# abdur75648/AI-Camera

Hardware: AMD Instinct MI355X
Metric: end-to-end frames/sec @1280x720, 30 persons/frame (higher is better)
Workload: dtype f16

## Files before the change

### ai-camera_amd/_lib.py

```python
from __future__ import annotations

import ctypes as C
import os

import numpy as np

HERE = os.path.dirname(os.path.abspath(__file__))
LIB_PATH = os.path.join(HERE, "libaicam.so")

OK, ERR_INVALID, ERR_NOT_FOUND, ERR_RUNTIME, ERR_NO_DEVICE, ERR_CAPACITY, ERR_FORMAT = 0, -1, -2, -3, -4, -5, -6
HOST, DEVICE = 0, 1
F32, F16 = 0, 1
MODEL_YOLO, MODEL_REID = 1, 2
PIX_BGR24, PIX_NV12, PIX_I420 = 0, 1, 2
YUV_BT601, YUV_BT709 = 0, 1
YUV_LIMITED, YUV_FULL = 0, 1
PROF_CLASSES = ("conv_igemm", "conv_direct", "misc", "letterbox", "crop_resize", "decode_nms", "tracker")


class AicError(RuntimeError):
    def __init__(self, code, msg):
        super().__init__(f"libaicam error {code}: {msg}")
        self.code = code

# ... 71 lines not shown
                ("max_persons", C.c_int32), ("conf_thresh", C.c_float), ("iou_thresh", C.c_float),
                ("max_det", C.c_int32), ("min_confidence", C.c_float), ("inject", C.c_int32),
                ("track_class_mask", C.c_uint64 * 2), ("tracker", TrackerParams)]


_P = C.c_void_p
_I = C.c_int
_F = C.c_float
_D = C.c_double
_SIGS = {
    "aic_last_error": (C.c_char_p, []),
    "aic_abi_version": (_I, []),
    "aic_device_count": (_I, [_P]),
    "aic_device_sync": (_I, [_I]),
    "aic_model_load": (_I, [C.c_char_p, _I, _I, _I, _P]),
    "aic_model_load_mem": (_I, [_P, C.c_size_t, _I, _I, _I, _P]),
    "aic_model_read_buffer": (_I, [_P, _I, _P, C.c_size_t]),
    "aic_model_conv_plan": (_I, [_P, _I, _I, _P]),
    "aic_model_conv_plan_live": (_I, [_P, _I, _I, _P]),
    "aic_model_row_band": (_I, [_P, _I, _I, _I, _P]),
    "aic_model_sparse_box": (_I, [_P, _I, _P]),
    "aic_debug_alloc_probe": (_I, [_I, _P, _P, _P, _P]),
    "aic_model_read_det": (_I, [_P, _I, _P, _P, _P]),
    "aic_detect_decode": (_I, [_P, _I, _I, _I, _F, _F, _I, _P, _P, _P, _P]),
    "aic_detect_live": (_I, [_P, _P, _I, _I, _I, _I, _I, _F, _F, _I, _P, _P, _P, _P]),
    "aic_model_destroy": (_I, [_P]),
    "aic_model_info": (_I, [_P, _P, _P, _P, _P, _P, _P, _P]),
    "aic_yolo_infer": (_I, [_P, _P, _I, _I, _F, _F, _I, _P, _P, _P, _P]),
    "aic_yolo_head": (_I, [_P, _P, _I, _I, _P, _P]),
    "aic_yolo_decode": (_I, [_P, _P, _I, _I, _P, _P, _P]),
    "aic_yolo_postprocess": (_I, [_P, _P, _P, _I, _F, _F, _I, _I, _F, _F, _F, _I, _I] + [_P] * 9),
    "aic_det_filter": (_I, [_I, _P, _P, _P, _P, _I, _I, _F, _P, _I] + [_P] * 9),
    "aic_reid_infer": (_I, [_P, _P, _I, _I, _P, _I]),
    "aic_reid_infer_live": (_I, [_P, _P, _I, _I, _I, _P, _I]),
    "aic_letterbox": (_I, [_I, _P, _I, _I, _I, _I, _P, _P, _P, _P]),
    "aic_letterbox_image": (_I, [_I, _P, _I, _I, _I, _I, _I, _I, _I, _I, _I, _I, _I, _P]),
    "aic_crop_resize": (_I, [_I, _P, _I, _I, _P, _I, _I, _I, _P, _P]),
    "aic_detect": (_I, [_P, _P, _I, _I, _I, _I, _F, _F, _I, _P, _P, _P, _P]),
    "aic_reid_embed": (_I, [_P, _P, _I, _I, _I, _P, _I, _P, _P]),
    "aic_crop_resize_ex": (_I, [_I, _P, _I, _I, _I, _I, _P, _P, _I, _I, _I, _I, _I, _I, _I, _P, _P]),
    "aic_reid_embed_bank": (_I, [_P, _P, _I, _I, _I, _I, _P, _P, _I, _I, _P, _P]),
    "aic_kf_initiate": (_I, [_I, _P, _I, _P, _P]),
    "aic_kf_predict": (_I, [_I, _P, _P, _I]),
    "aic_kf_predict_dt": (_I, [_I, _P, _P, _I, _F]),
    "aic_kf_project": (_I, [_I, _P, _P, _I, _P, _P]),
    "aic_kf_update": (_I, [_I, _P, _P, _P, _I]),
    "aic_kf_gating": (_I, [_I, _P, _P, _I, _P, _I, _I, _I, _P]),
    "aic_iou_cost": (_I, [_I, _P, _I, _P, _I, _P]),
    "aic_appearance_cost": (_I, [_I, _P, _P, _I, _I, _I, _P, _P, _I, _P]),
    "aic_lsap": (_I, [_P, _I, _I, _P, _P]),
    "aic_min_cost_matching": (_I, [_P, _I, _I, _D, _P, _P, _P]),
    "aic_match_cascade": (_I, [_P, _P, _P, _I, _I, _P, _P, _D, _D, _I, _P, _P, _P, _P, _P, _P, _P]),
    "aic_match_cascade_device": (_I, [_I, _P, _P, _P, _I, _I, _P, _P, _D, _D, _I, _I, _P, _P]),
    "aic_tracker_option": (_I, [_P, C.c_char_p, _I]),
    "aic_tracker_create": (_I, [_I, _P, _P]),
    "aic_tracker_destroy": (_I, [_P]),
    "aic_tracker_predict": (_I, [_P]),
    "aic_tracker_update": (_I, [_P, _P, _P, _P, _P, _I, _P, _I, _I]),
    "aic_tracker_update_batch": (_I, [_P, _I, _P, _P, _P, _P, _P, _I, _P, _I, _I, _P, _P, _P, _P, _P, _P]),
    "aic_tracker_import_state": (_I, [_P, _I, _P, _P, _P, _P, _P, _P, _P, _P, _P, _P, _P, _I, _I]),
    "aic_tracker_next_track_id": (_I, [_P, _P]),
    "aic_tracker_assoc_counters": (_I, [_P, _P, _P]),
    "aic_tracker_outputs": (_I, [_P, _P, _P, _I, _P]),
    "aic_tracker_num_tracks": (_I, [_P, _P]),
    "aic_tracker_export": (_I, [_P, _I, _P, _P, _P, _P, _P, _P, _P, _P, _P, _P]),
    "aic_tracker_export_gallery": (_I, [_P, _I, _P, _I]),
    "aic_tracker_last_matches": (_I, [_P, _P, _P, _I, _P]),
    "aic_tracker_last_costs": (_I, [_P, _P, _P, _P, _I, _P, _P]),
    "aic_pipeline_create": (_I, [_P, _P, _P, _P]),
    "aic_pipeline_destroy": (_I, [_P]),
    "aic_pipeline_upload": (_I, [_P, _I, _P, _I]),
    "aic_pipeline_inject": (_I, [_P, _I, _I, _P, _P, _P, _P]),
    "aic_pipeline_run": (_I, [_P, _I, _I, _P, _P, _P, _P, _P, _P, _P]),
    "aic_pipeline_run_passes": (_I, [_P, _I, _I, _I, _P, _P, _P, _P]),
    "aic_pipeline_run_from_host": (_I, [_P, _P, _I, _I, _P, _P, _P, _P]),
    "aic_pipeline_run_from_host_passes": (_I, [_P, _P, _I, _I, _I, _P, _P, _P, _P]),
    "aic_pipeline_group_times": (_I, [_P, _P, _P, _P, _I, _P]),
    "aic_pipeline_exchange_enable": (_I, [_P, _P, _P, _I, _I]),
    "aic_pipeline_exchange_stream": (_I, [_P, _P]),
    "aic_pipeline_exchange_wait": (_I, [_P, C.c_int64, _I, _P, _P]),
    "aic_pipeline_exchange_done": (_I, [_P, C.c_int64]),
    "aic_gallery_annotate": (_I, [_I, _P, _P, _I, _I, _I, _I, _D, _P, _P, _P, _P]),
    "aic_gid_create": (_I, [_I, _P]),
    "aic_gid_destroy": (_I, [_P]),
    "aic_gid_update": (_I, [_P, _I, _I, _P, _P, _P, _D, _P]),
    "aic_gid_lookup": (_I, [_P, _I, _I, _P]),
    "aic_gid_size": (_I, [_P, _P, _P, _P]),
    "aic_host_register": (_I, [_P, C.c_size_t]),
    "aic_host_unregister": (_I, [_P]),
    "aic_pipeline_tracker": (_I, [_P, _P]),
    "aic_pipeline_stats": (_I, [_P, _P, _P, _P, _P, _I]),
    "aic_pipeline_last_embeddings": (_I, [_P, _P, _I, _P, _P]),
    "aic_pipeline_option": (_I, [_P, C.c_char_p, _I]),
    "aic_pipeline_counters": (_I, [_P, _P, _P]),
    "aic_pipeline_assoc_frames": (_I, [_P, _P, _P]),
    "aic_pipeline_filter_counters": (_I, [_P, _P, _P, _P]),
    "aic_pipeline_lane_groups": (_I, [_P, _P]),
    "aic_pipeline_group_embeddings": (_I, [_P, _P, _I, _P, _I, _P, _P, _P]),
    "aic_overlay": (_I, [_I, _P, _I, _I, _I, _P, _I, _P, _I]),
    "aic_prof_enable": (_I, [_I, _I]),
    "aic_prof_reset": (_I, [_I]),
    "aic_prof_read": (_I, [_I, _I, _P, _P, _P, _P]),
    "aic_prof_read_union": (_I, [_I, _I, _P]),
    "aic_bytetrack_create": (_I, [_I, _P, _P]),
    "aic_bytetrack_destroy": (_I, [_P]),
    "aic_bytetrack_option": (_I, [_P, C.c_char_p, _I]),
# ... 239 lines not shown
```

### ai-camera_amd/csrc/kernels_trk_dev.hip

```cpp
#include "kernels.hpp"
#include "trk_dev.hpp"
#include "trk_math.hpp"
#include "trk_wave.hpp"

#include <algorithm>
#include <cstdio>
#include <cstdlib>

namespace aic {

namespace {

constexpr float kInfty = 1e5f;
constexpr float kChi2_4 = (float)9.487729036781154;
constexpr float kBig = 3.0e38f;

}

constexpr int SMG = 7;

__global__ __launch_bounds__(256) void trk_epoch_prep_kernel(const DevTrkHdr* __restrict__ hdr, const DevTrack* __restrict__ trk,
                                                             const float* __restrict__ gal_n, int gmax, int dim,
                                                             const float* __restrict__ featn, int dn, int dn_pad, int k,
                                                             float* __restrict__ sm, float* __restrict__ gram, int f0, EpochBankArgs bk) {
// ... 70 lines not shown
                        floatx4 a[4];
#pragma unroll
                        for (int u = 0; u < 4; ++u) a[u] = *reinterpret_cast<const floatx4*>(grow[g] + k0 + 16 * u + 4 * q);
#pragma unroll
                        for (int u = 0; u < 4; ++u)
#pragma unroll
                            for (int e = 0; e < 4; ++e) {
                                acc[g][0] = __builtin_amdgcn_mfma_f32_16x16x4f32(a[u][e], b0[u][e], acc[g][0], 0, 0, 0);
                                acc[g][1] = __builtin_amdgcn_mfma_f32_16x16x4f32(a[u][e], b1[u][e], acc[g][1], 0, 0, 0);
                            }
                    }
                }
            }
            for (; k0 < dim; k0 += 16) {
                const int kk = k0 + 4 * q;
                floatx4 b0 = {0.f, 0.f, 0.f, 0.f}, b1 = b0;
#pragma unroll
                for (int e = 0; e < 4; ++e)
                    if (kk + e < dim) { b0[e] = pa[kk + e]; b1[e] = pb[kk + e]; }
#pragma unroll
                for (int g = 0; g < SMG; ++g) {
                    if (g < ng) {
                        floatx4 a = {0.f, 0.f, 0.f, 0.f};
#pragma unroll
                        for (int e = 0; e < 4; ++e)
                            if (kk + e < dim) a[e] = grow[g][kk + e];
#pragma unroll
                        for (int e = 0; e < 4; ++e) {
                            acc[g][0] = __builtin_amdgcn_mfma_f32_16x16x4f32(a[e], b0[e], acc[g][0], 0, 0, 0);
                            acc[g][1] = __builtin_amdgcn_mfma_f32_16x16x4f32(a[e], b1[e], acc[g][1], 0, 0, 0);
                        }
                    }
                }
            }
#pragma unroll
            for (int g = SMG - 1; g >= 0; --g) {
                if (g < ng) {
#pragma unroll
                    for (int e = 0; e < 4; ++e) {
                        tile[4 * q + e][r] = cos_dist(acc[g][0][e]);
                        tile[4 * q + e][16 + r] = cos_dist(acc[g][1][e]);
                    }
                    wave_lds_sync();
                    if (lane < 32) {
                        for (int jj = 15; jj >= 0; --jj) {
                            const int row = 16 * (gb + g) + jj;
                            if (row < glen0) {
                                R = fminf(R, tile[jj][lane]);
                                if (row <= k) smt[(size_t)row * dn_pad + lane] = R;
                            }
                        }
                    }
                    wave_lds_sync();
                }
            }
        }
    }
}

namespace {

struct Lds {
    int *id, *state, *hits, *age, *tsu, *cls, *slot, *glen, *ghead, *sm, *napp, *glen0;
    float* conf;
    unsigned short* newrow;
    int ks;
    int *mdet;
    int *feas;
    float* tbox;
    int* free_slots;
    float *tlwh, *xyah, *dconf;
    int *dcls, *dhas, *mtrk, *und, *cols;
    int* rows;
    double *u, *v, *dist;
    int *pred, *rowof, *colof, *todo, *pos, *asg;
    int* wcnt;
    float* kf;
    float* arena;
    int arena_floats;
};

constexpr int KF_SLOTS = 96;

__device__ __forceinline__ Lds lds_carve(char* base, int cap, int nmax, int total_bytes, int ks = TRK_KMAX) {
    Lds L;
    char* p = base;
    auto take = [&](size_t bytes) { char* q = p; p += (bytes + 15) & ~(size_t)15; return q; };
    const size_t tc = (size_t)cap, mx = (size_t)max(cap, nmax);
    L.u = (double*)take(8 * mx); L.v = (double*)take(8 * mx); L.dist = (double*)take(8 * mx);
    int** ti[] = {&L.id, &L.state, &L.hits, &L.age, &L.tsu, &L.cls, &L.slot, &L.glen, &L.ghead, &L.sm, &L.napp, &L.glen0, &L.mdet, &L.rows, &L.feas};
    for (auto a : ti) *a = (int*)take(4 * tc);
    int** li[] = {&L.pred, &L.rowof, &L.colof, &L.todo, &L.pos, &L.asg};
    for (auto a : li) *a = (int*)take(4 * mx);
    L.conf = (float*)take(4 * tc);
    L.tbox = (float*)take(16 * tc);
    L.ks = ks;
    L.newrow = (unsigned short*)take(2 * tc * (size_t)ks);
    L.free_slots = (int*)take(4 * tc);
    L.kf = (float*)take(4 * 72 * (size_t)KF_SLOTS);
    L.tlwh = (float*)take(16 * (size_t)nmax); L.xyah = (float*)take(16 * (size_t)nmax); L.dconf = (float*)take(4 * (size_t)nmax);
    int** di[] = {&L.dcls, &L.dhas, &L.mtrk, &L.und, &L.cols};
    for (auto a : di) *a = (int*)take(4 * (size_t)nmax);
    L.wcnt = (int*)take(4 * (NW + 8));
    L.arena = (float*)p;
    L.arena_floats = (int)((total_bytes - (p - base)) / 4);
    return L;
// ... 858 lines not shown
    unsigned long long best = ~0ull;
    for (int j = tid; j < n; j += 256) {
        if (j / t_max == ri) continue;
        const float* gj = g + (size_t)j * w;
        if (!(gj[0] > 0.5f)) continue;
        float dot = 0.f;
        int k = 0;
        for (; k + 2 <= dim; k += 2) {
            const float2 b = *reinterpret_cast<const float2*>(gj + 2 + k);
            dot = dot + s_e[k] * b.x;
            dot = dot + s_e[k + 1] * b.y;
        }
        for (; k < dim; ++k) dot = dot + s_e[k] * gj[2 + k];
        const float d = cos_dist(dot);
        const unsigned long long key = ((unsigned long long)__float_as_uint(d) << 32) | (unsigned)j;
        best = key < best ? key : best;
    }
#pragma unroll
    for (int o = 32; o > 0; o >>= 1) {
        const unsigned long long other = __shfl_xor(best, o);
        best = other < best ? other : best;
    }
    if (lane == 0) s_best[wv] = best;
    __syncthreads();
    if (tid == 0) {
        unsigned long long b = s_best[0];
        for (int q = 1; q < 4; ++q) b = s_best[q] < b ? s_best[q] : b;
        near_row[i] = b == ~0ull ? -1 : (int)(unsigned)b;
        near_dist[i] = b == ~0ull ? kInfty : __uint_as_float((unsigned)(b >> 32));
    }
}

void launch_gallery_nearest(const float* gathered, int world, int t_max, int dim, int* ids, int* near_row, float* near_dist, hipStream_t s) {
    if (world * t_max <= 0) return;
    hipLaunchKernelGGL(gallery_nearest_kernel, dim3(world * t_max), dim3(256), (size_t)dim * 4, s, gathered, world, t_max, dim, ids, near_row, near_dist);
    KCHECK();
}

void launch_gallery_shard(const DevTrkHdr* hdr, const DevTrack* trk, const float* gal_n, int gmax, int dim, float* out, int t_max, hipStream_t s) {
    hipLaunchKernelGGL(gallery_shard_kernel, dim3(1), dim3(TRK_DEV_TMAX), 0, s, hdr, trk, gal_n, gmax, dim, out, t_max);
    KCHECK();
}

__global__ __launch_bounds__(256) void gallery_commit_kernel(const int* __restrict__ appends, const float* __restrict__ feat, const float* __restrict__ feat_n,
                                                             int d_begin, int dim, int gmax, float* __restrict__ gal_raw, float* __restrict__ gal_n,
                                                             size_t gal_stride) {
    appends += (size_t)blockIdx.y * TRK_APPENDS_INTS;
    gal_raw += blockIdx.y * gal_stride, gal_n += blockIdx.y * gal_stride;
    const int na = min(appends[3 * TRK_DEV_DNMAX], TRK_DEV_DNMAX), d4 = dim >> 2;
    const floatx4* fr = reinterpret_cast<const floatx4*>(feat + (size_t)d_begin * dim);
    const floatx4* fn = reinterpret_cast<const floatx4*>(feat_n + (size_t)d_begin * dim);
    floatx4* graw = reinterpret_cast<floatx4*>(gal_raw);
    floatx4* gn = reinterpret_cast<floatx4*>(gal_n);
    for (int i = blockIdx.x; i < na; i += gridDim.x) {
        const int slot = appends[i * 3], pos = appends[i * 3 + 1], er = appends[i * 3 + 2];
        const size_t dst = ((size_t)slot * gmax + pos) * d4, src = (size_t)er * d4;
        for (int c = threadIdx.x; c < 2 * d4; c += 256) {
            if (c < d4) graw[dst + c] = fr[src + c];
            else gn[dst + c - d4] = fn[src + c - d4];
        }
    }
}

static int epoch_lds_bytes() { return 159 * 1024; }

void launch_trk_epoch_prep(const DevTrkHdr* hdr, const DevTrack* trk, const float* gal_n, int gmax, int dim, int cap, const float* featn,
                           int dn, int dn_pad, int k, float* sm, float* gram, hipStream_t s) {
    if (dn <= 0) return;
    const long tasks = ((long)cap + dn_pad / 16) * (dn_pad / 32);
    const long likely = ((long)dn_pad / std::max(k, 1) + dn_pad / 16) * (dn_pad / 32);
    const int grid = (int)std::min<long>(std::min<long>(512, (tasks + 3) / 4), std::max<long>(64, likely / 9));
    hipLaunchKernelGGL(trk_epoch_prep_kernel, dim3(grid), dim3(256), 0, s, hdr, trk, gal_n, gmax, dim, featn, dn, dn_pad, k, sm, gram, 0, EpochBankArgs{});
    KCHECK();
}

void launch_trk_epoch_prep_bank(const EpochBankArgs& bk, int streams, const float* gal_n, int gmax, int dim, int cap, const float* featn,
                                int dn_pad_max, int f0, int k, float* sm, float* gram, hipStream_t s) {
    if (dn_pad_max <= 0 || streams <= 0) return;
    const long tasks = ((long)cap + dn_pad_max / 16) * (dn_pad_max / 32);
    const long likely = ((long)dn_pad_max / std::max(k, 1) + dn_pad_max / 16) * (dn_pad_max / 32);
    const long per = std::min<long>(std::min<long>(512, (tasks + 3) / 4), std::max<long>(64, likely / 9));
    const int grid = (int)std::max<long>(std::min<long>(per, std::max<long>(8, 1024 / streams)), 1);
    hipLaunchKernelGGL(trk_epoch_prep_kernel, dim3(grid, streams), dim3(256), 0, s, (const DevTrkHdr*)nullptr, (const DevTrack*)nullptr, gal_n, gmax,
                       dim, featn, 0, 0, k, sm, gram, f0, bk);
    KCHECK();
}

static void epoch_attr() {
    set_lds_limit(trk_epoch_kernel<false>, epoch_lds_bytes());
    set_lds_limit(trk_epoch_kernel<true>, epoch_lds_bytes());
    set_lds_limit(trk_cascade_test_kernel, epoch_lds_bytes());
}

namespace {
struct PhaseProf {
    long long* d = nullptr;
    long launches = 0, frames = 0;
    PhaseProf() {
        if (getenv("AICAM_TRK_PHASES")) { (void)hipMalloc((void**)&d, 16 * 8); (void)hipMemset(d, 0, 16 * 8); }
    }
    ~PhaseProf() {
        if (!d) return;
        long long h[16];
        (void)hipDeviceSynchronize();
        if (hipMemcpy(h, d, sizeof(h), hipMemcpyDeviceToHost) != hipSuccess || !frames) return;
        static const char* nm[8] = {"load table", "dets+predict", "cost rows", "cascade", "IoU stage", "lifecycle+KF update", "outputs+prune", "epoch tail"};
        fprintf(stderr, "[trk_phases] %ld epoch launches, %ld frames; shader cycles per frame:", launches, frames);
        for (int i = 0; i < 8; ++i) fprintf(stderr, " %s %.0f |", nm[i], (double)h[i] / frames);
        fprintf(stderr, "\n[trk_phases] inside the cascade: level search %.0f | row list %.0f | sub-matrix %.0f | unique-optimum check %.0f | unmatched list (+ the LSAP when the check fails) %.0f\n",
                (double)h[8] / frames, (double)h[9] / frames, (double)h[10] / frames, (double)h[11] / frames, (double)h[12] / frames);
        fprintf(stderr, "[trk_phases] assignment problems: %lld read off as the unique optimum, %lld through the LSAP\n", h[13], h[14]);
    }
};
PhaseProf g_phase;
}

void launch_trk_epoch(DevTrkHdr* hdr, DevTrack* trk, int* free_slots, float* mean, float* cov, float* gal_raw, float* gal_n,
                      const TrkDevParams& prm, const EpochDets& dets, int f0, int k, int d_begin, int dn_pad, int nmax, int has_sm,
                      const EpochScratch& scr, const EpochOut& out, hipStream_t s) {
    AIC_REQUIRE(prm.cap <= TRK_DEV_TMAX && nmax <= TRK_DEV_NMAX && k >= 1 && k <= TRK_KMAX, AIC_ERR_CAPACITY, "device association: shape beyond the epoch kernel");
    epoch_attr();
    EpochArgs a;
    a.hdr = hdr, a.trk = trk, a.free_slots = free_slots, a.mean = mean, a.cov = cov, a.gal_raw = gal_raw, a.gal_n = gal_n;
    a.prm = prm, a.dets = dets, a.f0 = f0, a.k = k, a.d_begin = d_begin, a.dn_pad = dn_pad, a.nmax = std::max(nmax, 1), a.has_sm = has_sm;
    a.scr = scr, a.out = out, a.lds_bytes = epoch_lds_bytes();
    a.commit_ext = (dets.feat != nullptr && dets.feat_n != nullptr && scr.appends != nullptr && prm.dim % 4 == 0) ? 1 : 0;
    a.prof = g_phase.d;
    a.cost_plane = TRK_DEV_TMAX * TRK_DEV_NMAX;
    a.bank = EpochBankArgs{};
    g_phase.launches += 1, g_phase.frames += k;
    hipLaunchKernelGGL(trk_epoch_kernel<false>, dim3(1), dim3(TRK_DEV_TMAX), (size_t)epoch_lds_bytes(), s, a);
    KCHECK();
    if (a.commit_ext) {
        hipLaunchKernelGGL(gallery_commit_kernel, dim3(256), dim3(256), 0, s, scr.appends, dets.feat, dets.feat_n, d_begin, prm.dim, prm.gmax, gal_raw, gal_n,
                           (size_t)0);
        KCHECK();
    }
}

void launch_trk_epoch_bank(const EpochBankArgs& bk, int streams, float* mean, float* cov, float* gal_raw, float* gal_n, const TrkDevParams& prm,
                           const EpochDets& dets, int f0, int k, int nmax_call, const EpochScratch& scr, const EpochOut& out, hipStream_t s) {
    AIC_REQUIRE(prm.cap <= TRK_DEV_TMAX && nmax_call <= TRK_DEV_NMAX && k >= 1 && k <= TRK_KMAX && streams >= 1, AIC_ERR_CAPACITY,
                "device association: shape beyond the epoch kernel");
    AIC_REQUIRE(bk.stream_k && bk.stream_f0 && bk.plan && bk.row_map && scr.appends && prm.dim % 4 == 0, AIC_ERR_INVALID, "device association: incomplete bank launch");
    epoch_attr();
    EpochArgs a{};
    a.mean = mean, a.cov = cov, a.gal_raw = gal_raw, a.gal_n = gal_n;
    a.prm = prm, a.dets = dets, a.f0 = f0, a.k = k, a.nmax = 1;
    a.scr = scr, a.out = out, a.lds_bytes = epoch_lds_bytes();
    a.commit_ext = 1;
    a.prof = g_phase.d;
    a.cost_plane = prm.cap * std::max(nmax_call, 1);
    a.bank = bk;
    g_phase.launches += 1, g_phase.frames += k;
    hipLaunchKernelGGL(trk_epoch_kernel<true>, dim3(streams), dim3(TRK_DEV_TMAX), (size_t)epoch_lds_bytes(), s, a);
    KCHECK();
    if (dets.feat != nullptr && dets.feat_n != nullptr) {
        hipLaunchKernelGGL(gallery_commit_kernel, dim3(std::max(8, 256 / streams), streams), dim3(256), 0, s, scr.appends, dets.feat, dets.feat_n, 0, prm.dim,
                           prm.gmax, gal_raw, gal_n, bk.gal_stride);
        KCHECK();
    }
}

void launch_trk_cascade_test(const TrkDevParams& prm, const EpochScratch& scr, int T, int n, const int* state, const int* tsu,
                             int* out_mdet, int* out_err, int stage1_only, hipStream_t s) {
    AIC_REQUIRE(T <= TRK_DEV_TMAX && n <= TRK_DEV_NMAX, AIC_ERR_CAPACITY, "device cascade: at most 512 tracks x 512 detections");
    epoch_attr();
    EpochArgs a{};
    a.prm = prm, a.scr = scr, a.nmax = std::max(n, 1), a.lds_bytes = epoch_lds_bytes();
    hipLaunchKernelGGL(trk_cascade_test_kernel, dim3(1), dim3(TRK_DEV_TMAX), (size_t)epoch_lds_bytes(), s, a, T, n, state, tsu, out_mdet, out_err,
                       epoch_lds_bytes(), stage1_only);
    KCHECK();
}

}
```

### ai-camera_amd/csrc/tracker.cpp

```cpp
#include "tracker.hpp"

#include <chrono>
#include <cstdio>

#include <algorithm>
#include <cmath>

namespace aic {

static const float kInfty = 1e5f;

Tracker::Tracker(Device& d, const aic_tracker_params& p) : dev(&d), prm(p) {
    cap = p.max_tracks > 0 ? p.max_tracks : 512;
    unlimited = p.nn_budget <= 0;
    gmax = unlimited ? 256 : p.nn_budget;
    next_id = p.first_track_id > 0 ? p.first_track_id : 1;
    d.use();
    d_mean.alloc((size_t)cap * 8);
    d_cov.alloc((size_t)cap * 64);
    for (int s = cap - 1; s >= 0; --s) free_slots.push_back(s);
    if (p.feature_dim > 0) ensure_dim(p.feature_dim);
}

void Tracker::ensure_dim(int d) {
// ... 817 lines not shown
        if (k == "device_assoc") {
            AIC_REQUIRE(!value || t->t.dev_capable(), AIC_ERR_INVALID,
                        "device association needs nn_budget > 0, max_tracks <= 512 and a feature dimension divisible by 4");
            if (!value) t->t.to_host();
            t->t.dev_assoc = value != 0;
        } else if (k == "wave_cascade") {
            t->t.wave_cascade = value != 0;
        } else if (k == "lsap_fast") {
            t->t.lsap_fast = value != 0;
        } else if (k == "epoch_frames") {
            AIC_REQUIRE(value >= 0 && value <= TRK_KMAX, AIC_ERR_INVALID, "epoch_frames must be in 0..16 (0 = default)");
            t->t.epoch_frames = value;
        } else AIC_REQUIRE(false, AIC_ERR_INVALID, "unknown tracker option: " + k);
    });
}

int aic_match_cascade_device(int device_id, const float* app, const float* maha, const float* iou, int t, int n, const int32_t* state,
                             const int32_t* tsu, double max_cosine_distance, double max_iou_distance, int max_age, int flags,
                             int32_t* match_det_of_track, int32_t* n_fast_lsap) {
    return guarded([&] {
        AIC_REQUIRE(t >= 0 && n >= 0 && t <= TRK_DEV_TMAX && n <= TRK_DEV_NMAX, AIC_ERR_CAPACITY, "at most 512 tracks x 512 detections");
        if (t == 0) return;
        AIC_REQUIRE(state && tsu && match_det_of_track && (n == 0 || (app && maha && iou)), AIC_ERR_INVALID, "NULL argument");
        Device& d = device(device_id);
        d.use();
        hipStream_t s = d.s_trk;
        const size_t stride = (size_t)TRK_DEV_TMAX * TRK_DEV_NMAX, tn = (size_t)t * n;
        DevBuf<float> costs(3 * stride), sub(stride);
        DevBuf<int> st(t), ts(t), md(t + 3);
        if (tn) {
            HIP_CHECK(hipMemcpyAsync(costs.p, app, tn * 4, hipMemcpyHostToDevice, s));
            HIP_CHECK(hipMemcpyAsync(costs.p + stride, maha, tn * 4, hipMemcpyHostToDevice, s));
            HIP_CHECK(hipMemcpyAsync(costs.p + 2 * stride, iou, tn * 4, hipMemcpyHostToDevice, s));
        }
        HIP_CHECK(hipMemcpyAsync(st.p, state, (size_t)t * 4, hipMemcpyHostToDevice, s));
        HIP_CHECK(hipMemcpyAsync(ts.p, tsu, (size_t)t * 4, hipMemcpyHostToDevice, s));
        TrkDevParams prm{};
        prm.max_cos = (float)max_cosine_distance, prm.clamp_cos = (float)(max_cosine_distance + 1e-5);
        prm.max_iou = (float)max_iou_distance, prm.clamp_iou = (float)(max_iou_distance + 1e-5);
        prm.max_age = max_age, prm.n_init = 3, prm.gmax = 1, prm.dim = 0, prm.cap = TRK_DEV_TMAX;
        prm.no_fast = (flags & 2) ? 1 : 0;
        prm.no_wave = (flags & 4) ? 1 : 0;
        EpochScratch scr{nullptr, nullptr, costs.p, sub.p, nullptr};
        launch_trk_cascade_test(prm, scr, t, n, st.p, ts.p, md.p, md.p + t, flags & 1, s);
        std::vector<int> out(t + 3);
        HIP_CHECK(hipMemcpyAsync(out.data(), md.p, (size_t)(t + 3) * 4, hipMemcpyDeviceToHost, s));
        HIP_CHECK(hipStreamSynchronize(s));
        AIC_REQUIRE(out[t] == 0, AIC_ERR_INVALID, "cost matrix contains NaN/-inf or is infeasible");
        std::copy(out.begin(), out.begin() + t, match_det_of_track);
        if (n_fast_lsap) { n_fast_lsap[0] = out[t + 1]; n_fast_lsap[1] = out[t + 2]; }
    });
}

int aic_tracker_predict(aic_tracker* t) {
    return guarded([&] {
        AIC_REQUIRE(t, AIC_ERR_INVALID, "NULL tracker");
        t->t.predict();
    });
}

int aic_tracker_update(aic_tracker* t, const float* det_tlwh, const float* conf, const int32_t* cls, const float* feat,
                       int feat_mem, const uint8_t* has_feat, int n, int dim) {
    return guarded([&] {
        AIC_REQUIRE(t, AIC_ERR_INVALID, "NULL tracker");
        AIC_REQUIRE(n == 0 || (det_tlwh && conf && cls), AIC_ERR_INVALID, "NULL detection arrays");
        t->t.update(det_tlwh, conf, cls, feat, feat_mem, has_feat, n, dim);
    });
}

int aic_tracker_update_batch(aic_tracker* t, int k, const int32_t* counts, const float* det_tlwh, const float* conf, const int32_t* cls,
                             const float* feat, int feat_mem, const uint8_t* has_feat, int dim, int cap_rows, int32_t* n_out, int32_t* out6,
                             float* out_conf, int32_t* n_match, int32_t* match_track_id, int32_t* match_det) {
    return guarded([&] {
        AIC_REQUIRE(t && (k == 0 || counts), AIC_ERR_INVALID, "NULL argument");
        long total = 0;
        for (int f = 0; f < k; ++f) total += counts[f];
        AIC_REQUIRE(total == 0 || (det_tlwh && conf && cls), AIC_ERR_INVALID, "NULL detection arrays");
        t->t.update_batch(k, counts, det_tlwh, conf, cls, feat, feat_mem, has_feat, dim, cap_rows, n_out, out6, out_conf, n_match, match_track_id, match_det);
    });
}

int aic_tracker_import_state(aic_tracker* t, int n, const int32_t* track_id, const int32_t* state, const int32_t* hits, const int32_t* age,
                             const int32_t* time_since_update, const int32_t* cls, const float* conf, const int32_t* gallery_len,
                             const float* mean, const float* cov, const float* galleries, int dim, int next_track_id) {
    return guarded([&] {
        AIC_REQUIRE(t, AIC_ERR_INVALID, "NULL tracker");
        t->t.import_state(n, track_id, state, hits, age, time_since_update, cls, conf, gallery_len, mean, cov, galleries, dim, next_track_id);
    });
}

int aic_tracker_next_track_id(aic_tracker* t, int32_t* next_id) {
    return guarded([&] {
        AIC_REQUIRE(t && next_id, AIC_ERR_INVALID, "NULL argument");
        t->t.to_host();
        *next_id = t->t.next_id;
    });
}

int aic_tracker_assoc_counters(aic_tracker* t, int64_t* n_fast, int64_t* n_lsap) {
    return guarded([&] {
        AIC_REQUIRE(t, AIC_ERR_INVALID, "NULL tracker");
        if (n_fast) *n_fast = t->t.n_fast;
        if (n_lsap) *n_lsap = t->t.n_lsap;
    });
}

// ... 99 lines not shown
```

### include/aicam.h

```cpp
#ifndef AICAM_H
#define AICAM_H

#include <stddef.h>
#include <stdint.h>

#ifdef __cplusplus
extern "C" {
#endif

#define AIC_ABI_VERSION 2

#define AIC_OK 0
#define AIC_ERR_INVALID (-1)
#define AIC_ERR_NOT_FOUND (-2)
#define AIC_ERR_RUNTIME (-3)
#define AIC_ERR_NO_DEVICE (-4)
#define AIC_ERR_CAPACITY (-5)
#define AIC_ERR_FORMAT (-6)

#define AIC_HOST 0
#define AIC_DEVICE 1

#define AIC_F32 0
#define AIC_F16 1
// ... 56 lines not shown
int aic_letterbox(int device, const uint8_t* frame_bgr, int h, int w, int out_h, int out_w,
                  float* out_nchw, float* ratio, float* pad_w, float* pad_h);
int aic_letterbox_image(int device, const uint8_t* frame_bgr, int h, int w, int unpad_h, int unpad_w, int top, int bottom,
                        int left, int right, int color_b, int color_g, int color_r, uint8_t* out_bgr);
int aic_crop_resize(int device, const uint8_t* frame_bgr, int h, int w, const float* boxes_xyxy,
                    int n, int out_h, int out_w, float* out_nchw, int32_t* valid);

int aic_detect(aic_model* yolo, const uint8_t* frames_bgr, int batch, int h, int w, int mem,
               float conf_thresh, float iou_thresh, int max_det, int32_t* num_dets, float* boxes_xyxy,
               float* scores, int32_t* labels);
int aic_detect_decode(aic_model* yolo, int batch, int h, int w, float conf_thresh, float iou_thresh, int max_det,
                      int32_t* num_dets, float* boxes_xyxy, float* scores, int32_t* labels);
int aic_detect_live(aic_model* yolo, const uint8_t* frames_bgr, int batch, int n_live, int h, int w, int mem,
                    float conf_thresh, float iou_thresh, int max_det, int32_t* num_dets, float* boxes_xyxy,
                    float* scores, int32_t* labels);

int aic_reid_embed(aic_model* reid, const uint8_t* frame_bgr, int h, int w, int mem,
                   const float* boxes_xyxy, int n, float* embeddings, int32_t* valid);

int aic_crop_resize_ex(int device, const uint8_t* frames_bgr, int n_frames, int h, int w, int byte_offset, const float* boxes_xyxy,
                       const int32_t* frame_of, int n, int n_live, int out_h, int out_w, int mode, int dtype, int slack, void* out,
                       int32_t* valid);
int aic_reid_embed_bank(aic_model* reid, const uint8_t* frames_bgr, int n_frames, int h, int w, int byte_offset,
                        const float* boxes_xyxy, const int32_t* frame_of, int n, int n_live, float* embeddings, int32_t* valid);
int aic_reid_infer_live(aic_model* m, const float* crops_nchw, int n, int n_live, int mem, float* embeddings, int out_mem);

int aic_kf_initiate(int device, const float* z, int n, float* mean, float* cov);
int aic_kf_predict(int device, float* mean, float* cov, int n);
int aic_kf_predict_dt(int device, float* mean, float* cov, int n, float dt);
int aic_kf_project(int device, const float* mean, const float* cov, int n, float* pmean, float* pcov);
int aic_kf_update(int device, float* mean, float* cov, const float* z, int n);
int aic_kf_gating(int device, const float* mean, const float* cov, int n, const float* zs, int m,
                  int shared_z, int only_position, float* d2);

int aic_iou_cost(int device, const float* track_tlwh, int t, const float* det_tlwh, int n, float* cost);
int aic_appearance_cost(int device, const float* galleries, const int32_t* gallery_len, int t,
                        int gmax, int dim, const float* det_feat, const uint8_t* has_feat, int n,
                        float* cost);

int aic_lsap(const double* cost, int nr, int nc, int64_t* row_ind, int64_t* col_ind);
int aic_min_cost_matching(const float* cost, int nr, int nc, double max_distance, int32_t* match_row,
                          int32_t* match_col, int32_t* n_match);

int aic_match_cascade(const float* app, const float* maha, const float* iou, int t, int n, const int32_t* state,
                      const int32_t* time_since_update, double max_cosine_distance, double max_iou_distance,
                      int max_age, int32_t* match_track, int32_t* match_det, int32_t* n_match,
                      int32_t* unmatched_tracks, int32_t* n_unmatched_tracks, int32_t* unmatched_dets,
                      int32_t* n_unmatched_dets);

int aic_match_cascade_device(int device, const float* app, const float* maha, const float* iou, int t, int n,
                             const int32_t* state, const int32_t* time_since_update, double max_cosine_distance,
                             double max_iou_distance, int max_age, int flags, int32_t* match_det_of_track,
                             int32_t* n_fast_lsap);

typedef struct aic_tracker_params {
    double max_cosine_distance;
    double max_iou_distance;
    int32_t nn_budget;
    int32_t max_age;
    int32_t n_init;
    int32_t max_tracks;
    int32_t feature_dim;
    int32_t first_track_id;
} aic_tracker_params;

int aic_tracker_create(int device, const aic_tracker_params* p, aic_tracker** out);
int aic_tracker_destroy(aic_tracker* t);
int aic_tracker_option(aic_tracker* t, const char* key, int value);
int aic_tracker_predict(aic_tracker* t);
int aic_tracker_update(aic_tracker* t, const float* det_tlwh, const float* conf, const int32_t* cls,
                       const float* feat, int feat_mem, const uint8_t* has_feat, int n, int dim);
int aic_tracker_update_batch(aic_tracker* t, int k, const int32_t* counts, const float* det_tlwh, const float* conf,
                             const int32_t* cls, const float* feat, int feat_mem, const uint8_t* has_feat, int dim,
                             int cap_rows, int32_t* n_out, int32_t* out6, float* out_conf, int32_t* n_match,
                             int32_t* match_track_id, int32_t* match_det);
int aic_tracker_outputs(aic_tracker* t, int32_t* out6, float* conf, int cap, int32_t* n_out);
int aic_tracker_num_tracks(const aic_tracker* t, int32_t* n);
int aic_tracker_export(aic_tracker* t, int cap, int32_t* track_id, int32_t* state, int32_t* hits,
                       int32_t* age, int32_t* time_since_update, int32_t* cls, float* conf,
                       int32_t* gallery_len, float* mean, float* cov);
int aic_tracker_export_gallery(aic_tracker* t, int index, float* out, int cap_rows);
int aic_tracker_next_track_id(aic_tracker* t, int32_t* next_id);
int aic_tracker_import_state(aic_tracker* t, int n, const int32_t* track_id, const int32_t* state, const int32_t* hits,
                             const int32_t* age, const int32_t* time_since_update, const int32_t* cls, const float* conf,
                             const int32_t* gallery_len, const float* mean, const float* cov, const float* galleries,
                             int dim, int next_track_id);
int aic_tracker_assoc_counters(aic_tracker* t, int64_t* n_unique, int64_t* n_lsap);
int aic_tracker_last_matches(aic_tracker* t, int32_t* track_id, int32_t* det, int cap, int32_t* n);
int aic_tracker_last_costs(aic_tracker* t, float* app, float* maha, float* iou, int cap, int32_t* t_n,
                           int32_t* d_n);

int aic_deepsort_bank_create(int device, const aic_tracker_params* p, int streams, aic_deepsort_bank** out);
int aic_deepsort_bank_destroy(aic_deepsort_bank* b);
int aic_deepsort_bank_option(aic_deepsort_bank* b, const char* key, int value);
int aic_deepsort_bank_update(aic_deepsort_bank* b, const int32_t* frames_per_stream, const int32_t* counts, const float* det_tlwh,
                             const float* conf, const int32_t* cls, const float* feat, const int32_t* valid, int cap_rows,
                             int32_t* n_out, int32_t* out6, float* out_conf, int32_t* status);
int aic_deepsort_bank_reset(aic_deepsort_bank* b, int stream);
int aic_deepsort_bank_export(aic_deepsort_bank* b, int stream, int cap, int32_t* track_id, int32_t* state, int32_t* hits,
                             int32_t* age, int32_t* time_since_update, int32_t* cls, float* conf, int32_t* gallery_len,
                             float* mean, float* cov, int32_t* n_tracks);
int aic_deepsort_bank_export_gallery(aic_deepsort_bank* b, int stream, int index, float* out, int cap_rows);
int aic_deepsort_bank_counters(aic_deepsort_bank* b, int stream, int64_t* n_unique, int64_t* n_lsap);

typedef struct aic_bytetrack_params {
    double track_thresh;
// ... 411 lines not shown
```

Before: 12650.

## Add blocked track-partitioned epoch prep kernel and size gallery commit grid to rows

Adds a second form of the tracker epoch prep kernel. Each block stages a 32-row detection tile in LDS and walks a strided subset of tracks in groups of eight, computing gallery-by-detection cosine tiles with f32 MFMA and software-pipelined register prefetch. Running minima go through LDS tiles, and the suffix-min rows are written at the end. It is used by default when the gallery fits (gmax ≤ 256, dim%4==0), and an env var falls back to the old form. The gallery commit kernel now assigns one wave per appended row and launches a grid sized to the row count rather than a fixed 256 blocks. A host test entry point and an env-controlled repeat loop are also added, at the cost of extra code paths and LDS pressure.

```diff
diff --git a/ai-camera_amd/_lib.py b/ai-camera_amd/_lib.py
--- a/ai-camera_amd/_lib.py
+++ b/ai-camera_amd/_lib.py
@@ -147,6 +147,7 @@
     "aic_min_cost_matching": (_I, [_P, _I, _I, _D, _P, _P, _P]),
     "aic_match_cascade": (_I, [_P, _P, _P, _I, _I, _P, _P, _D, _D, _I, _P, _P, _P, _P, _P, _P, _P]),
     "aic_match_cascade_device": (_I, [_I, _P, _P, _P, _I, _I, _P, _P, _D, _D, _I, _I, _P, _P]),
+    "aic_trk_prep_test": (_I, [_I, _I, _I, _P, _P, _P, _I, _I, _P, _I, _P, _P, _P, _I, _I, _P, _P]),
     "aic_tracker_option": (_I, [_P, C.c_char_p, _I]),
     "aic_tracker_create": (_I, [_I, _P, _P]),
     "aic_tracker_destroy": (_I, [_P]),
diff --git a/ai-camera_amd/csrc/kernels_trk_dev.hip b/ai-camera_amd/csrc/kernels_trk_dev.hip
--- a/ai-camera_amd/csrc/kernels_trk_dev.hip
+++ b/ai-camera_amd/csrc/kernels_trk_dev.hip
@@ -146,6 +146,198 @@
                         }
                     }
                     wave_lds_sync();
+                }
+            }
+        }
+    }
+}
+
+constexpr int PREP_NTB = 8;
+constexpr int PREP_GCAP = 16;
+constexpr int PREP_TG = TRK_KMAX / 16 + 1;
+
+static size_t prep2_lds_bytes(int dim) {
+    return ((size_t)32 * (dim + 4) + (size_t)PREP_NTB * PREP_TG * 16 * 36 + PREP_NTB * 4 * 32) * 4 + (3 * PREP_NTB + PREP_NTB * PREP_GCAP + 4) * 4;
+}
+
+__global__ __launch_bounds__(256) void trk_epoch_prep2_kernel(const DevTrkHdr* __restrict__ hdr, const DevTrack* __restrict__ trk,
+                                                              const float* __restrict__ gal_n, int gmax, int dim,
+                                                              const float* __restrict__ featn, int dn, int dn_pad, int k,
+                                                              float* __restrict__ sm, float* __restrict__ gram, int f0, int P, EpochBankArgs bk) {
+    extern __shared__ floatx4 prep_lds[];
+    const int tid = threadIdx.x, wv = tid >> 6, lane = tid & 63, r = lane & 15, q = lane >> 4;
+    const int pitch = dim + 4;
+    float* bst = reinterpret_cast<float*>(prep_lds);
+    float* tiles = bst + 32 * pitch;
+    float* rest = tiles + PREP_NTB * PREP_TG * 16 * 36;
+    int* l_slot = reinterpret_cast<int*>(rest + PREP_NTB * 4 * 32);
+    int* l_glen = l_slot + PREP_NTB;
+    int* l_ghead = l_glen + PREP_NTB;
+    int* utab = l_ghead + PREP_NTB;
+    const int* rmap = nullptr;
+    if (bk.stream_k) {
+        const size_t sid = blockIdx.y;
+        const EpochStreamPlan pl = bk.plan[sid];
+        hdr = reinterpret_cast<const DevTrkHdr*>(bk.tbl + sid * bk.tbl_stride);
+        if (!pl.has_sm || bk.stream_k[sid] <= f0 || hdr->err) return;
+        trk = reinterpret_cast<const DevTrack*>(hdr + 1);
+        gal_n += sid * bk.gal_stride, sm += sid * bk.sm_stride, gram += sid * bk.gram_stride;
+        dn = pl.dn, dn_pad = pl.dn_pad;
+        rmap = bk.row_map + pl.map0;
+    }
+    auto frow = [&](int i) -> const float* { return featn + (size_t)(rmap ? rmap[i] : i) * dim; };
+    const int T0 = hdr->n_tracks;
+    const int c = blockIdx.x / P, p = blockIdx.x - c * P;
+    if (c >= dn_pad / 32) return;
+    const int d_base = c * 32;
+    const int ngr = 2 * c + 1 >= p ? (2 * c + 1 - p) / P + 1 : 0;
+    const int ntr = T0 > p ? (T0 - p + P - 1) / P : 0;
+    if (ngr == 0 && ntr == 0) return;
+    {
+        const int d4 = dim >> 2;
+        for (int row = wv; row < 32; row += 4) {
+            const floatx4* src = reinterpret_cast<const floatx4*>(frow(min(d_base + row, dn - 1)));
+            floatx4* dst = reinterpret_cast<floatx4*>(bst + row * pitch);
+            for (int i = lane; i < d4; i += 64) dst[i] = src[i];
+        }
+    }
+    const float* bA = bst + r * pitch + 4 * q;
+    const float* bB = bst + (16 + r) * pitch + 4 * q;
+    const int ns = dim / 64;
+    for (int t0 = 0; t0 == 0 || t0 < ntr; t0 += PREP_NTB) {
+        const int nt = max(0, min(PREP_NTB, ntr - t0));
+        __syncthreads();
+        if (tid < nt) {
+            const DevTrack* tr = trk + p + (size_t)(t0 + tid) * P;
+            l_slot[tid] = tr->slot, l_glen[tid] = tr->glen, l_ghead[tid] = tr->ghead;
+        }
+        for (int i = tid; i < PREP_NTB * 4 * 32; i += 256) rest[i] = kBig;
+        __syncthreads();
+        int nsm = 0;
+        {
+            const int tl = tid / PREP_GCAP, g = tid - tl * PREP_GCAP;
+            int before = 0;
+            for (int i = 0; i < nt; ++i) {
+                const int G = min((l_glen[i] + 15) / 16, PREP_GCAP);
+                if (i < tl) before += G;
+                if (i == tl && g < G) utab[before + g] = tl << 8 | g;
+                nsm += G;
+            }
+        }
+        __syncthreads();
+        const int nu = nsm + (t0 == 0 ? ngr : 0);
+        auto unit_a = [&](int u) -> const float* {
+            if (u >= nsm) return frow(min((p + (u - nsm) * P) * 16 + r, dn - 1));
+            const int e = utab[u], tl = e >> 8;
+            const int j = min(16 * (e & 255) + r, l_glen[tl] - 1);
+            int pos = l_ghead[tl] + j;
+            if (pos >= gmax) pos -= gmax;
+            return gal_n + ((size_t)l_slot[tl] * gmax + pos) * dim;
+        };
+        floatx4 a[4], b0[4], b1[4], a2[4], b20[4], b21[4];
+        const float* gp = wv < nu ? unit_a(wv) : nullptr;
+        if (gp && ns > 0) {
+#pragma unroll
+            for (int v = 0; v < 4; ++v) {
+                a[v] = *reinterpret_cast<const floatx4*>(gp + 16 * v + 4 * q);
+                b0[v] = *reinterpret_cast<const floatx4*>(bA + 16 * v);
+                b1[v] = *reinterpret_cast<const floatx4*>(bB + 16 * v);
+            }
+        }
+        for (int u = wv; u < nu; u += 4) {
+            const float* gpn = u + 4 < nu ? unit_a(u + 4) : gp;
+            floatx4 acc0 = {0.f, 0.f, 0.f, 0.f}, acc1 = acc0;
+            auto slice = [&](int s, const floatx4 (&ca)[4], const floatx4 (&cb0)[4], const floatx4 (&cb1)[4], floatx4 (&na)[4], floatx4 (&nb0)[4],
+                             floatx4 (&nb1)[4]) {
+                const bool wrap = s + 1 == ns;
+                const float* an_p = (wrap ? gpn : gp + 64 * (s + 1)) + 4 * q;
+                const int kb = wrap ? 0 : 64 * (s + 1);
+#pragma unroll
+                for (int v = 0; v < 4; ++v) {
+                    na[v] = *reinterpret_cast<const floatx4*>(an_p + 16 * v);
+                    nb0[v] = *reinterpret_cast<const floatx4*>(bA + kb + 16 * v);
+                    nb1[v] = *reinterpret_cast<const floatx4*>(bB + kb + 16 * v);
+                }
+                __builtin_amdgcn_sched_barrier(0);
+#pragma unroll
+                for (int v = 0; v < 4; ++v)
+#pragma unroll
+                    for (int e = 0; e < 4; ++e) {
+                        acc0 = __builtin_amdgcn_mfma_f32_16x16x4f32(ca[v][e], cb0[v][e], acc0, 0, 0, 0);
+                        acc1 = __builtin_amdgcn_mfma_f32_16x16x4f32(ca[v][e], cb1[v][e], acc1, 0, 0, 0);
+                    }
+                __builtin_amdgcn_sched_barrier(0);
+            };
+            int s = 0;
+            for (; s + 2 <= ns; s += 2) {
+                slice(s, a, b0, b1, a2, b20, b21);
+                slice(s + 1, a2, b20, b21, a, b0, b1);
+            }
+            if (s < ns) {
+                slice(s, a, b0, b1, a2, b20, b21);
+#pragma unroll
+                for (int v = 0; v < 4; ++v) a[v] = a2[v], b0[v] = b20[v], b1[v] = b21[v];
+            }
+            for (int k0 = ns * 64; k0 < dim; k0 += 16) {
+                const int kk = k0 + 4 * q;
+                floatx4 ta = {0.f, 0.f, 0.f, 0.f}, tb0 = ta, tb1 = ta;
+#pragma unroll
+                for (int e = 0; e < 4; ++e)
+                    if (kk + e < dim) { ta[e] = gp[kk + e]; tb0[e] = bA[k0 + e]; tb1[e] = bB[k0 + e]; }
+#pragma unroll
+                for (int e = 0; e < 4; ++e) {
+                    acc0 = __builtin_amdgcn_mfma_f32_16x16x4f32(ta[e], tb0[e], acc0, 0, 0, 0);
+                    acc1 = __builtin_amdgcn_mfma_f32_16x16x4f32(ta[e], tb1[e], acc1, 0, 0, 0);
+                }
+            }
+            if (u >= nsm) {
+                const int a0 = (p + (u - nsm) * P) * 16;
+#pragma unroll
+                for (int e = 0; e < 4; ++e) {
+                    float* o = gram + (size_t)(a0 + 4 * q + e) * dn_pad + d_base;
+                    o[r] = cos_dist(acc0[e]);
+                    o[16 + r] = cos_dist(acc1[e]);
+                }
+            } else {
+                const int en = utab[u], tl = en >> 8, g = en & 255;
+                if (16 * g <= k) {
+                    float* tile = tiles + (tl * PREP_TG + g) * 16 * 36;
+#pragma unroll
+                    for (int e = 0; e < 4; ++e) {
+                        tile[(4 * q + e) * 36 + r] = cos_dist(acc0[e]);
+                        tile[(4 * q + e) * 36 + 16 + r] = cos_dist(acc1[e]);
+                    }
+                } else {
+                    float m0, m1;
+                    cos_tile_min(acc0, acc1, 16 * g, q, l_glen[tl], m0, m1);
+                    float* rw = rest + (tl * 4 + wv) * 32;
+                    if (q == 0) {
+                        rw[r] = fminf(rw[r], m0);
+                        rw[16 + r] = fminf(rw[16 + r], m1);
+                    }
+                    wave_lds_sync();
+                }
+            }
+            gp = gpn;
+        }
+        __syncthreads();
+        if (lane < 32) {
+            for (int tl = wv; tl < nt; tl += 4) {
+                const int glen0 = l_glen[tl];
+                float* smt = sm + ((size_t)p + (size_t)(t0 + tl) * P) * (TRK_KMAX + 1) * dn_pad + d_base;
+                for (int e = glen0; e <= k; ++e) smt[(size_t)e * dn_pad + lane] = kBig;
+                const float* rw = rest + tl * 4 * 32;
+                float R = fminf(fminf(rw[lane], rw[32 + lane]), fminf(rw[64 + lane], rw[96 + lane]));
+                const int G = min((glen0 + 15) / 16, PREP_GCAP);
+                for (int g = min(G, k / 16 + 1) - 1; g >= 0; --g) {
+                    const float* tile = tiles + (tl * PREP_TG + g) * 16 * 36;
+                    for (int jj = 15; jj >= 0; --jj) {
+                        const int row = 16 * g + jj;
+                        if (row < glen0) {
+                            R = fminf(R, tile[jj * 36 + lane]);
+                            if (row <= k) smt[(size_t)row * dn_pad + lane] = R;
+                        }
+                    }
                 }
             }
         }
@@ -1110,21 +1302,47 @@
     const floatx4* fn = reinterpret_cast<const floatx4*>(feat_n + (size_t)d_begin * dim);
     floatx4* graw = reinterpret_cast<floatx4*>(gal_raw);
     floatx4* gn = reinterpret_cast<floatx4*>(gal_n);
-    for (int i = blockIdx.x; i < na; i += gridDim.x) {
+    const int wv = threadIdx.x >> 6, lane = threadIdx.x & 63;
+    for (int i = blockIdx.x * 4 + wv; i < na; i += gridDim.x * 4) {
         const int slot = appends[i * 3], pos = appends[i * 3 + 1], er = appends[i * 3 + 2];
         const size_t dst = ((size_t)slot * gmax + pos) * d4, src = (size_t)er * d4;
-        for (int c = threadIdx.x; c < 2 * d4; c += 256) {
+        for (int c = lane; c < 2 * d4; c += 64) {
             if (c < d4) graw[dst + c] = fr[src + c];
             else gn[dst + c - d4] = fn[src + c - d4];
         }
     }
 }
 
+static int commit_blocks(long rows, int most) { return (int)std::max<long>(1, std::min<long>(most, (std::min<long>(rows, TRK_DEV_DNMAX) + 3) / 4)); }
+
 static int epoch_lds_bytes() { return 159 * 1024; }
+
+static bool prep_second_form(int gmax, int dim) {
+    static const bool v1 = [] { const char* e = getenv("AICAM_TRK_PREP_V1"); return e && atoi(e) != 0; }();
+    if (v1 || dim % 4 != 0 || gmax > 16 * PREP_GCAP || prep2_lds_bytes(dim) > (size_t)160 * 1024) return false;
+    set_lds_limit(trk_epoch_prep2_kernel, (size_t)160 * 1024);
+    return true;
+}
+
+static int prep2_split(int gmax, int dn_pad, int k, long most) {
+    const int groups = std::max(1, (gmax + 15) / 16), per_block = std::max(1, 36 / groups);
+    const long likely = std::max(1, dn_pad / std::max(k, 1));
+    return (int)std::max<long>(1, std::min<long>((likely + per_block - 1) / per_block, most / (dn_pad / 32)));
+}
 
 void launch_trk_epoch_prep(const DevTrkHdr* hdr, const DevTrack* trk, const float* gal_n, int gmax, int dim, int cap, const float* featn,
                            int dn, int dn_pad, int k, float* sm, float* gram, hipStream_t s) {
     if (dn <= 0) return;
+    static const int repeat = [] { const char* e = getenv("AICAM_TRK_PREP_REPEAT"); return e ? std::max(1, std::min(atoi(e), 16)) : 1; }();
+    if (prep_second_form(gmax, dim)) {
+        const int P = prep2_split(gmax, dn_pad, k, 512);
+        for (int i = 0; i < repeat; ++i) {
+            hipLaunchKernelGGL(trk_epoch_prep2_kernel, dim3(dn_pad / 32 * P), dim3(256), prep2_lds_bytes(dim), s, hdr, trk, gal_n, gmax, dim, featn, dn, dn_pad, k,
+                               sm, gram, 0, P, EpochBankArgs{});
+            KCHECK();
+        }
+        return;
+    }
     const long tasks = ((long)cap + dn_pad / 16) * (dn_pad / 32);
     const long likely = ((long)dn_pad / std::max(k, 1) + dn_pad / 16) * (dn_pad / 32);
     const int grid = (int)std::min<long>(std::min<long>(512, (tasks + 3) / 4), std::max<long>(64, likely / 9));
@@ -1135,6 +1353,13 @@
 void launch_trk_epoch_prep_bank(const EpochBankArgs& bk, int streams, const float* gal_n, int gmax, int dim, int cap, const float* featn,
                                 int dn_pad_max, int f0, int k, float* sm, float* gram, hipStream_t s) {
     if (dn_pad_max <= 0 || streams <= 0) return;
+    if (prep_second_form(gmax, dim)) {
+        const int P = prep2_split(gmax, dn_pad_max, k, std::max<long>(8, 1024 / streams));
+        hipLaunchKernelGGL(trk_epoch_prep2_kernel, dim3(dn_pad_max / 32 * P, streams), dim3(256), prep2_lds_bytes(dim), s, (const DevTrkHdr*)nullptr,
+                           (const DevTrack*)nullptr, gal_n, gmax, dim, featn, 0, 0, k, sm, gram, f0, P, bk);
+        KCHECK();
+        return;
+    }
     const long tasks = ((long)cap + dn_pad_max / 16) * (dn_pad_max / 32);
     const long likely = ((long)dn_pad_max / std::max(k, 1) + dn_pad_max / 16) * (dn_pad_max / 32);
     const long per = std::min<long>(std::min<long>(512, (tasks + 3) / 4), std::max<long>(64, likely / 9));
@@ -1190,7 +1415,7 @@
     hipLaunchKernelGGL(trk_epoch_kernel<false>, dim3(1), dim3(TRK_DEV_TMAX), (size_t)epoch_lds_bytes(), s, a);
     KCHECK();
     if (a.commit_ext) {
-        hipLaunchKernelGGL(gallery_commit_kernel, dim3(256), dim3(256), 0, s, scr.appends, dets.feat, dets.feat_n, d_begin, prm.dim, prm.gmax, gal_raw, gal_n,
+        hipLaunchKernelGGL(gallery_commit_kernel, dim3(commit_blocks(dn_pad, 256)), dim3(256), 0, s, scr.appends, dets.feat, dets.feat_n, d_begin, prm.dim, prm.gmax, gal_raw, gal_n,
                            (size_t)0);
         KCHECK();
     }
@@ -1214,7 +1439,7 @@
     hipLaunchKernelGGL(trk_epoch_kernel<true>, dim3(streams), dim3(TRK_DEV_TMAX), (size_t)epoch_lds_bytes(), s, a);
     KCHECK();
     if (dets.feat != nullptr && dets.feat_n != nullptr) {
-        hipLaunchKernelGGL(gallery_commit_kernel, dim3(std::max(8, 256 / streams), streams), dim3(256), 0, s, scr.appends, dets.feat, dets.feat_n, 0, prm.dim,
+        hipLaunchKernelGGL(gallery_commit_kernel, dim3(commit_blocks((long)std::max(nmax_call, 1) * k, std::max(8, 256 / streams)), streams), dim3(256), 0, s, scr.appends, dets.feat, dets.feat_n, 0, prm.dim,
                            prm.gmax, gal_raw, gal_n, bk.gal_stride);
         KCHECK();
     }
diff --git a/ai-camera_amd/csrc/tracker.cpp b/ai-camera_amd/csrc/tracker.cpp
--- a/ai-camera_amd/csrc/tracker.cpp
+++ b/ai-camera_amd/csrc/tracker.cpp
@@ -893,6 +893,73 @@
     });
 }
 
+int aic_trk_prep_test(int device_id, int streams, int cap, const int32_t* n_tracks, const int32_t* slot_glen_ghead, const float* gal_n, int gmax,
+                      int dim, const float* feat_n, int rows, const int32_t* stream_dn, const int32_t* row_map, const int32_t* has_sm, int k,
+                      int dn_pad, float* sm, float* gram) {
+    return guarded([&] {
+        AIC_REQUIRE(n_tracks && slot_glen_ghead && gal_n && feat_n && stream_dn && sm && gram, AIC_ERR_INVALID, "NULL argument");
+        AIC_REQUIRE(streams >= 0 && streams <= 64 && cap >= 1 && cap <= TRK_DEV_TMAX && gmax >= 1 && dim >= 4 && dim % 4 == 0 && rows >= 1 && k >= 1 &&
+                    k <= TRK_KMAX && dn_pad >= 32 && dn_pad % 32 == 0 && dn_pad <= TRK_DEV_DNMAX, AIC_ERR_INVALID, "prep test: shape out of range");
+        const int S = std::max(streams, 1);
+        AIC_REQUIRE(streams == 0 || (row_map && has_sm), AIC_ERR_INVALID, "prep test: a bank needs row_map and has_sm");
+        const size_t tbl_stride = sizeof(DevTrkHdr) + (size_t)cap * sizeof(DevTrack) + (size_t)cap * 4;
+        std::vector<char> tbl(tbl_stride * S, 0);
+        std::vector<EpochStreamPlan> plan(S);
+        std::vector<int> sk(S, k);
+        int map_n = 0;
+        for (int s = 0; s < S; ++s) {
+            AIC_REQUIRE(n_tracks[s] >= 0 && n_tracks[s] <= cap, AIC_ERR_INVALID, "prep test: n_tracks out of range");
+            DevTrkHdr* h = reinterpret_cast<DevTrkHdr*>(tbl.data() + tbl_stride * s);
+            DevTrack* tr = reinterpret_cast<DevTrack*>(h + 1);
+            h->n_tracks = n_tracks[s];
+            for (int i = 0; i < n_tracks[s]; ++i) {
+                const int32_t* e = slot_glen_ghead + ((size_t)s * cap + i) * 3;
+                AIC_REQUIRE(e[0] >= 0 && e[0] < cap && e[1] >= 0 && e[1] <= gmax && e[2] >= 0 && e[2] < gmax, AIC_ERR_INVALID, "prep test: track out of range");
+                tr[i].slot = e[0], tr[i].glen = e[1], tr[i].ghead = e[2];
+            }
+            const int dn = stream_dn[s];
+            AIC_REQUIRE(dn >= (streams ? 0 : 1) && dn <= dn_pad && (streams || dn <= rows), AIC_ERR_INVALID, "prep test: detection rows out of range");
+            plan[s] = EpochStreamPlan{};
+            plan[s].dn = dn, plan[s].dn_pad = std::max(32, (dn + 31) / 32 * 32), plan[s].nmax = 1, plan[s].map0 = map_n;
+            plan[s].has_sm = streams ? (has_sm[s] && dn > 0) : 1;
+            if (streams) {
+                for (int i = 0; i < dn; ++i) AIC_REQUIRE(row_map[map_n + i] >= 0 && row_map[map_n + i] < rows, AIC_ERR_INVALID, "prep test: row_map out of range");
+                map_n += dn;
+            }
+        }
+        AIC_REQUIRE(streams || plan[0].dn_pad == dn_pad, AIC_ERR_INVALID, "prep test: dn_pad must be the padded row count");
+        Device& d = device(device_id);
+        d.use();
+        hipStream_t st = d.s_trk;
+        const size_t gal_stride = (size_t)cap * gmax * dim, sm_stride = (size_t)cap * (TRK_KMAX + 1) * dn_pad, gram_stride = (size_t)dn_pad * dn_pad;
+        DevBuf<char> d_tbl(tbl.size());
+        DevBuf<float> d_gal(gal_stride * S), d_feat((size_t)rows * dim), d_sm(sm_stride * S), d_gram(gram_stride * S);
+        DevBuf<EpochStreamPlan> d_plan(S);
+        DevBuf<int> d_sk(S), d_map(std::max(map_n, 1));
+        std::vector<float> fill(std::max(sm_stride, gram_stride) * S, -1.0f);
+        HIP_CHECK(hipMemcpyAsync(d_tbl.p, tbl.data(), tbl.size(), hipMemcpyHostToDevice, st));
+        HIP_CHECK(hipMemcpyAsync(d_gal.p, gal_n, gal_stride * S * 4, hipMemcpyHostToDevice, st));
+        HIP_CHECK(hipMemcpyAsync(d_feat.p, feat_n, (size_t)rows * dim * 4, hipMemcpyHostToDevice, st));
+        HIP_CHECK(hipMemcpyAsync(d_sm.p, fill.data(), sm_stride * S * 4, hipMemcpyHostToDevice, st));
+        HIP_CHECK(hipMemcpyAsync(d_gram.p, fill.data(), gram_stride * S * 4, hipMemcpyHostToDevice, st));
+        HIP_CHECK(hipMemcpyAsync(d_plan.p, plan.data(), sizeof(EpochStreamPlan) * S, hipMemcpyHostToDevice, st));
+        HIP_CHECK(hipMemcpyAsync(d_sk.p, sk.data(), (size_t)S * 4, hipMemcpyHostToDevice, st));
+        if (map_n) HIP_CHECK(hipMemcpyAsync(d_map.p, row_map, (size_t)map_n * 4, hipMemcpyHostToDevice, st));
+        if (streams) {
+            EpochBankArgs bk{};
+            bk.tbl = d_tbl.p, bk.tbl_stride = tbl_stride, bk.gal_stride = gal_stride, bk.sm_stride = sm_stride, bk.gram_stride = gram_stride;
+            bk.stream_k = d_sk.p, bk.plan = d_plan.p, bk.row_map = d_map.p;
+            launch_trk_epoch_prep_bank(bk, S, d_gal.p, gmax, dim, cap, d_feat.p, dn_pad, 0, k, d_sm.p, d_gram.p, st);
+        } else {
+            launch_trk_epoch_prep(reinterpret_cast<const DevTrkHdr*>(d_tbl.p), reinterpret_cast<const DevTrack*>(d_tbl.p + sizeof(DevTrkHdr)), d_gal.p, gmax,
+                                  dim, cap, d_feat.p, stream_dn[0], dn_pad, k, d_sm.p, d_gram.p, st);
+        }
+        HIP_CHECK(hipMemcpyAsync(sm, d_sm.p, sm_stride * S * 4, hipMemcpyDeviceToHost, st));
+        HIP_CHECK(hipMemcpyAsync(gram, d_gram.p, gram_stride * S * 4, hipMemcpyDeviceToHost, st));
+        HIP_CHECK(hipStreamSynchronize(st));
+    });
+}
+
 int aic_tracker_predict(aic_tracker* t) {
     return guarded([&] {
         AIC_REQUIRE(t, AIC_ERR_INVALID, "NULL tracker");
diff --git a/include/aicam.h b/include/aicam.h
--- a/include/aicam.h
+++ b/include/aicam.h
@@ -132,6 +132,10 @@
                              const int32_t* state, const int32_t* time_since_update, double max_cosine_distance,
                              double max_iou_distance, int max_age, int flags, int32_t* match_det_of_track,
                              int32_t* n_fast_lsap);
+
+int aic_trk_prep_test(int device, int streams, int cap, const int32_t* n_tracks, const int32_t* slot_glen_ghead,
+                      const float* gal_n, int gmax, int dim, const float* feat_n, int rows, const int32_t* stream_dn,
+                      const int32_t* row_map, const int32_t* has_sm, int k, int dn_pad, float* sm, float* gram);
 
 typedef struct aic_tracker_params {
     double max_cosine_distance;
```

Result: faster. 12800, median of 6 (+1.2%).
